# guptakhil/show-tell

Measured on AMD Instinct MI355X. Metric: training images/sec (ResNet101+GRU, emb=512, bs=128) at 1/2/4/8 MI355X, higher is better.
Workload: dtype bf16; 1 GPU; BASELINE configs[1]: ResNet-101 (train-mode BN, frozen) + 5-layer GRU decoder, E=H=512, V=10000, fwd+bwd+SGD step, synthetic COCO-shaped batch; batch_per_gpu=128, global_batch=128, image=3x224x224, parallelism=dp1

## Files before the change

### include/showtell_hip.h

```cpp
#ifndef SHOWTELL_HIP_H
#define SHOWTELL_HIP_H

#include <stddef.h>
#include <stdint.h>

#ifdef __cplusplus
extern "C" {
#endif

#define ST_F32 0
#define ST_BF16 1

#define ST_CELL_GRU 0
#define ST_CELL_LSTM 1

const char* st_last_error(void);
int st_version(void);

typedef struct {
  const void* x;
  const void* w;
  void* y;
  const float* bias;
  const float* scale;
// ... 110 lines not shown
  const void* x_s2d; const void* w_frag; void* y;
  float* stats; int stats_replicas;
  const float* gamma;
  const float* scale; const float* shift;
  int B, H, W;
} st_stem_conv_pool_desc;
int st_stem_conv_pool(const st_stem_conv_pool_desc* d, void* stream);
int st_stem_weight_frag(const void* w_s2d, void* out, void* stream);
int st_stem_weight_frag_packed(const void* w_packed, int Cpad, void* out, void* stream);
int st_global_avgpool(const void* x, void* y, int dtype, int out_dtype, int B, int HW, int C, void* stream);

typedef struct st_image_batch_desc {
  const uint8_t* src;
  int64_t src_bytes;
  const int64_t* offset;
  const int32_t* height;
  const int32_t* width;
  const int32_t* flip;
  int batch;
  int max_height, max_width;
  int out_h, out_w;
  const float* lut;
  uint8_t* tmp;
  float* out;
  uint8_t* out_u8;
} st_image_batch_desc;
int st_image_transform(const st_image_batch_desc* d, void* stream);

int st_cast(const void* x, void* y, int from_dtype, int to_dtype, long n, void* stream);
int st_transpose(const void* x, void* y, int dtype, int rows, int cols, int ldx, int ldy, void* stream);
int st_transpose_colsum(const void* x, void* y, float* colsum, int dtype, int rows, int cols, int ldx, int ldy, void* stream);
int st_transpose_batch(const void* const* x, void* const* y, float* const* colsum, int n, int dtype, int rows, int cols,
                       int ldx, int ldy, const int* rows_t, const int* prev_row, void* stream);
int st_pack_conv_weight(const float* w, void* out, int dtype, int Cout, int Cin, int KH, int KW, int Cpad, int k_order, void* stream);

typedef struct st_resnet st_resnet;
int st_resnet_create(int version, int dtype, st_resnet** out);
void st_resnet_destroy(st_resnet* r);
int st_resnet_num_convs(const st_resnet* r);
int st_resnet_feat_dim(const st_resnet* r);
size_t st_resnet_weight_elems(const st_resnet* r);
size_t st_resnet_bn_channels(const st_resnet* r);
int st_resnet_conv_info(const st_resnet* r, int i, int* cin, int* cout, int* k, int* stride, int* pad,
                        int* cin_padded, size_t* weight_offset, size_t* bn_offset, int* k_order,
                        size_t* frag_weight_offset, int* frag_ntw);
size_t st_resnet_workspace_bytes(const st_resnet* r, int B, int H, int W);
int st_resnet_set_taps(st_resnet* r, void* buf, size_t bytes);
int st_resnet_forward(const st_resnet* r, const float* images_nchw, int B, int H, int W,
                      const void* weights, const float* bn_gamma, const float* bn_beta,
                      float* bn_running_mean, float* bn_running_var,
                      int train, float momentum, float eps,
                      void* workspace, size_t workspace_bytes,
                      void* feat_nhwc_out, void* pooled_out, int pooled_dtype, float* ncp_out,
                      void* stream);

int st_resnet_update_running(const st_resnet* r, const void* workspace, float* bn_running_mean, float* bn_running_var,
                             float momentum, void* stream);
int st_resnet_plan(const st_resnet* r, int B, int H, int W, int train, char* buf, size_t bytes);

int st_cast2d(const void* x, void* y, int from_dtype, int to_dtype, int rows, int cols, int ldx, int ldy, void* stream);

#define ST_MAX_LAYERS 8
typedef struct {
  int cell, dtype, L, in0, H, V, E;
  const void* emb;
  const void* w_ih[ST_MAX_LAYERS]; const void* w_hh[ST_MAX_LAYERS];
// ... 115 lines not shown
```

### show-tell_amd/_lib.py

```python
import ctypes as C
import os

_HERE = os.path.dirname(os.path.abspath(__file__))
LIB_PATH = os.path.join(_HERE, "lib", "libshowtell_hip.so")

ST_F32, ST_BF16 = 0, 1
ST_CELL_GRU, ST_CELL_LSTM = 0, 1

c_p, c_i, c_f, c_l = C.c_void_p, C.c_int, C.c_float, C.c_long


class ConvDesc(C.Structure):
    _fields_ = [("x", c_p), ("w", c_p), ("y", c_p), ("bias", c_p), ("scale", c_p), ("shift", c_p),
                ("residual", c_p), ("stats", c_p), ("dtype", c_i), ("out_dtype", c_i),
                ("B", c_i), ("Hin", c_i), ("Win", c_i), ("Cin", c_i), ("Ho", c_i), ("Wo", c_i), ("N", c_i),
                ("KH", c_i), ("KW", c_i), ("stride", c_i), ("pad", c_i),
                ("ldx", c_i), ("ldw", c_i), ("ldy", c_i), ("relu", c_i), ("accumulate", c_i), ("Cin_logical", c_i), ("k_order", c_i), ("stats_replicas", c_i),
                ("in_stats", c_p), ("in_gamma", c_p), ("in_beta", c_p), ("in_count", c_f), ("in_eps", c_f), ("split_k", c_i)]


class Conv3x3ImgDesc(C.Structure):
    _fields_ = [("x", c_p), ("w_frag", c_p), ("y", c_p), ("stats", c_p), ("stats_replicas", c_i), ("scale", c_p), ("shift", c_p),
                ("relu", c_i), ("in_stats", c_p), ("in_gamma", c_p), ("in_beta", c_p), ("in_count", c_f), ("in_eps", c_f),
                ("B", c_i), ("H", c_i), ("W", c_i), ("C", c_i), ("N", c_i), ("in_stats_replicas", c_i)]
# ... 43 lines not shown
                ("res_beta", c_p), ("res_running_mean", c_p), ("res_running_var", c_p), ("res_bn", c_i),
                ("dtype", c_i), ("rows", c_l), ("C", c_i), ("count", c_f), ("eps", c_f), ("relu", c_i),
                ("stats_replicas", c_i), ("res_stats_replicas", c_i)]


ST_MAX_LAYERS = 8


class RnnParams(C.Structure):
    _fields_ = [("cell", c_i), ("dtype", c_i), ("L", c_i), ("in0", c_i), ("H", c_i), ("V", c_i), ("E", c_i),
                ("emb", c_p), ("w_ih", c_p * ST_MAX_LAYERS), ("w_hh", c_p * ST_MAX_LAYERS),
                ("b_ih", c_p * ST_MAX_LAYERS), ("b_hh", c_p * ST_MAX_LAYERS), ("w_lin", c_p), ("b_lin", c_p)]


class RnnGrads(C.Structure):
    _fields_ = [("emb", c_p), ("w_ih", c_p * ST_MAX_LAYERS), ("w_hh", c_p * ST_MAX_LAYERS),
                ("b_ih", c_p * ST_MAX_LAYERS), ("b_hh", c_p * ST_MAX_LAYERS), ("w_lin", c_p), ("b_lin", c_p)]


class AttnParams(C.Structure):
    _fields_ = [("rnn", RnnParams), ("F", c_i), ("A", c_i), ("P", c_i),
                ("w_enc", c_p), ("b_enc", c_p), ("w_dec", c_p), ("b_dec", c_p), ("w_full", c_p), ("b_full", c_p),
                ("w_init_h", c_p), ("b_init_h", c_p), ("w_init_c", c_p), ("b_init_c", c_p), ("w_embed", c_p), ("b_embed", c_p)]


class AttnGrads(C.Structure):
    _fields_ = [("rnn", RnnGrads)] + [(n, c_p) for n in ("w_enc", "b_enc", "w_dec", "b_dec", "w_full", "b_full", "w_init_h", "b_init_h",
                                                        "w_init_c", "b_init_c", "w_embed", "b_embed")]


class PackedSeq(C.Structure):
    _fields_ = [("B", c_i), ("T", c_i), ("ntok", c_i), ("Tcap", c_i), ("batch_sizes_host", C.POINTER(c_i)),
                ("rows_b", c_p), ("rows_t", c_p), ("prev_row", c_p), ("caption", c_p)]


class ImageBatchDesc(C.Structure):
    _fields_ = [("src", c_p), ("src_bytes", C.c_int64), ("offset", c_p), ("height", c_p), ("width", c_p), ("flip", c_p), ("batch", c_i),
                ("max_height", c_i), ("max_width", c_i), ("out_h", c_i), ("out_w", c_i), ("lut", c_p), ("tmp", c_p),
                ("out", c_p), ("out_u8", c_p)]


_SIGS = {
    "st_version": ([], c_i),
    "st_image_transform": ([C.POINTER(ImageBatchDesc), c_p], c_i),
    "st_conv": ([C.POINTER(ConvDesc), c_p], c_i),
    "st_conv_batch": ([C.POINTER(ConvDesc), c_i, c_p], c_i),
    "st_conv3x3_img_supported": ([c_i, c_i, c_i, c_i], c_i),
    "st_conv3x3_img": ([C.POINTER(Conv3x3ImgDesc), c_p], c_i),
    "st_conv3x3_s2_supported": ([c_i, c_i], c_i),
    "st_conv3x3_s2": ([C.POINTER(Conv3x3ImgDesc), c_p], c_i),
    "st_conv1x1_wreg_supported": ([c_i, c_i], c_i),
    "st_conv1x1_wreg": ([C.POINTER(Conv1x1WregDesc), c_p], c_i),
    "st_conv1x1_kfuse": ([C.POINTER(Conv1x1KfuseDesc), c_p], c_i),
    "st_conv1x1_kfuse_supported": ([c_i, c_i], c_i),
    "st_conv1x1_kfuse8": ([C.POINTER(Conv1x1KfuseDesc), c_p], c_i),
    "st_conv_b2b": ([C.POINTER(ConvB2bDesc), c_p], c_i),
    "st_conv_b2b_supported": ([c_i, c_i, c_i], c_i),
    "st_conv1x1_astat_supported": ([c_i, c_i], c_i),
    "st_conv1x1_astat": ([C.POINTER(Conv1x1WregDesc), c_p], c_i),
    "st_conv1x1_kstream_supported": ([c_i, c_i], c_i),
    "st_conv1x1_kstream": ([C.POINTER(Conv1x1WregDesc), c_p], c_i),
    "st_pack_conv_weight_frag": ([c_p, c_p, c_i, c_i, c_i, c_i, c_i, c_p], c_i),
    "st_tune": ([c_i, c_i, c_i], c_i),
    "st_prof_enable": ([c_i], c_i),
    "st_debug_stamps": ([c_p], c_i),
    "st_prof_collect": ([C.POINTER(C.c_double), C.POINTER(C.c_double), C.POINTER(c_l)], c_i),
    "st_bn_act": ([C.POINTER(BnActDesc), c_p], c_i),
    "st_bn_update_running": ([c_p, c_p, c_p, c_i, c_f, c_f, c_p], c_i),
    "st_nchw_to_nhwc": ([c_p, c_p, c_i, c_i, c_i, c_i, c_i, c_i, c_p], c_i),
    "st_nchw_to_s2d16": ([c_p, c_p, c_i, c_i, c_i, c_i, c_p], c_i),
    "st_stem_weight_s2d": ([c_p, c_p, c_i, c_i, c_p], c_i),
    "st_stem_weight_frag": ([c_p, c_p, c_p], c_i),
    "st_stem_weight_frag_packed": ([c_p, c_i, c_p, c_p], c_i),
    "st_stem_conv_pool": ([C.POINTER(StemConvPoolDesc), c_p], c_i),
    "st_nhwc_to_ncp_f32": ([c_p, c_p, c_i, c_i, c_i, c_i, c_p], c_i),
    "st_maxpool3x3s2": ([c_p, c_p, c_i, c_i, c_i, c_i, c_i, c_p], c_i),
    "st_maxpool3x3s2_bn": ([c_p, c_p, c_i, c_i, c_i, c_i, c_i, c_p, c_p, c_p, c_p, c_p, c_f, c_f, c_p], c_i),
    "st_global_avgpool": ([c_p, c_p, c_i, c_i, c_i, c_i, c_i, c_p], c_i),
    "st_cast": ([c_p, c_p, c_i, c_i, c_l, c_p], c_i),
    "st_transpose": ([c_p, c_p, c_i, c_i, c_i, c_i, c_i, c_p], c_i),
    "st_transpose_colsum": ([c_p, c_p, c_p, c_i, c_i, c_i, c_i, c_i, c_p], c_i),
    "st_transpose_batch": ([c_p, c_p, c_p, c_i, c_i, c_i, c_i, c_i, c_i, c_p, c_p, c_p], c_i),
    "st_pack_conv_weight": ([c_p, c_p, c_i, c_i, c_i, c_i, c_i, c_i, c_i, c_p], c_i),
    "st_cast2d": ([c_p, c_p, c_i, c_i, c_i, c_i, c_i, c_i, c_p], c_i),
    "st_rnn_vocab_ld": ([c_i], c_i),
    "st_rnn_workspace_bytes": ([C.POINTER(RnnParams), C.POINTER(PackedSeq)], C.c_size_t),
    "st_rnn_forward": ([C.POINTER(RnnParams), C.POINTER(PackedSeq), c_p, c_p, c_p, C.c_size_t, c_p, c_i, c_i, c_p, c_i, c_p], c_i),
    "st_rnn_fused_loss_supported": ([C.POINTER(RnnParams)], c_i),
    "st_rnn_fused_loss_bytes": ([C.POINTER(RnnParams), C.POINTER(PackedSeq)], C.c_size_t),
    "st_rnn_fused_loss": ([C.POINTER(RnnParams), C.POINTER(PackedSeq), c_p, C.c_size_t, c_p, c_p, C.c_size_t, c_p, c_p], c_i),
    "st_rnn_fused_dlogits": ([C.POINTER(RnnParams), C.POINTER(PackedSeq), c_p, C.c_size_t, c_p, c_p, c_p, c_p, c_i, c_p], c_i),
    "st_rnn_backward": ([C.POINTER(RnnParams), C.POINTER(RnnGrads), C.POINTER(PackedSeq), c_p, c_p, c_i, c_p, c_p, C.c_size_t,
                         c_p, c_p, c_p], c_i),
    "st_rnn_greedy_workspace_bytes": ([C.POINTER(RnnParams), c_i], C.c_size_t),
    "st_rnn_greedy": ([C.POINTER(RnnParams), c_p, c_i, c_i, c_p, C.c_size_t, c_p, c_p, c_p], c_i),
    "st_rnn_greedy_last_route": ([], c_i),
    "st_rnn_step": ([C.POINTER(RnnParams), c_p, c_i, c_p, c_p, c_p, c_p, c_p, c_i, c_p], c_i),
    "st_embedding_rows": ([c_p, c_p, c_p, c_i, c_i, c_i, c_i, c_i, c_p], c_i),
    "st_gather_state": ([c_p, c_p, c_p, c_i, c_i, c_i, c_i, c_i, c_p], c_i),
    "st_softmax_topk": ([c_p, c_i, c_i, c_i, c_i, c_p, c_p, c_i, c_p], c_i),
    "st_beam_select": ([c_p, c_p, c_p, c_p, c_p, c_i, c_i, c_i, c_l, c_p, c_p, c_p, c_p, c_p, c_p], c_i),
    "st_sample_rows": ([c_p, c_i, c_i, c_i, c_p, c_i, c_f, c_i, c_l, c_p, c_p, c_p, c_i, c_i, c_p, c_p], c_i),
    "st_rnn_sample_workspace_bytes": ([C.POINTER(RnnParams), c_i], C.c_size_t),
    "st_rnn_sample": ([C.POINTER(RnnParams), c_p, c_i, c_i, c_p, c_f, c_i, c_l, c_p, C.c_size_t, c_p, c_p, c_p], c_i),
    "st_attn_workspace_bytes": ([c_p, c_p], C.c_size_t),
    "st_attn_forward": ([c_p, c_p, c_p, c_p, c_p, C.c_size_t, c_p, c_i, c_i, c_p, c_i, c_p], c_i),
    "st_attn_backward": ([c_p, c_p, c_p, c_p, c_p, c_i, c_p, c_p, c_f, c_p, c_p, C.c_size_t, c_p], c_i),
    "st_attn_reg_loss": ([c_p, c_i, c_i, c_i, c_f, c_p, c_p], c_i),
    "st_attn_greedy_workspace_bytes": ([c_p, c_i], C.c_size_t),
    "st_attn_greedy": ([c_p, c_p, c_i, c_i, c_l, c_p, C.c_size_t, c_p, c_p], c_i),
    "st_attn_greedy_alphas": ([c_p, c_p, c_i, c_i, c_l, c_p, C.c_size_t, c_p, c_p, c_p], c_i),
    "st_attn_sample_workspace_bytes": ([c_p, c_i], C.c_size_t),
    "st_attn_sample": ([c_p, c_p, c_i, c_i, c_l, c_p, c_f, c_i, c_l, c_p, C.c_size_t, c_p, c_p, c_p, c_p], c_i),
    "st_attn_beam_workspace_bytes": ([c_p, c_i, c_i], C.c_size_t),
    "st_attn_beam_search": ([c_p, c_p, c_i, c_i, c_i, c_l, c_l, c_p, C.c_size_t, c_p, c_p, c_p, c_p, c_p, c_p], c_i),
# ... 63 lines not shown
```

### show-tell_amd/csrc/rnn.cpp

```cpp
#include "decoder_host.h"
#include <stdlib.h>

namespace {

struct Plan {
  int G, GH, Np, Vp, maxw;
  size_t es;
  size_t x0, y, gates, cst, dyl, dx0, dgx, dgh, dhc, dcc, tA, tB, wT, wThh, wTih, gA, gB, total;
};

Plan make_plan(const st_rnn_params* p, const st_packed_seq* s) {
  Plan q;
  q.G = p->cell == ST_CELL_GRU ? 3 : 4;
  q.GH = q.G * p->H;
  q.Np = st_up8(s->ntok);
  q.Vp = st_rnn_vocab_ld(p->V);
  q.es = st_dtype_size(p->dtype);
  q.maxw = p->in0 > p->H ? p->in0 : p->H;
  const size_t n = s->ntok, L = p->L, H = p->H;
  Arena ar;
  q.x0 = ar.take(n * p->in0 * q.es);
  q.y = ar.take(L * n * H * q.es);
  q.gates = ar.take(L * n * 4 * H * q.es);
  q.cst = ar.take(p->cell == ST_CELL_LSTM ? L * n * H * q.es : 0);
  q.dyl = ar.take(L * n * H * sizeof(float));
  q.dx0 = ar.take(n * p->in0 * sizeof(float));
  q.dgx = ar.take(L * n * q.GH * q.es);
  q.dgh = ar.take(p->cell == ST_CELL_GRU ? L * n * q.GH * q.es : 0);
  q.dhc = ar.take(L * (size_t)s->B * H * sizeof(float));
  q.dcc = ar.take(L * (size_t)s->B * H * sizeof(float));
  const size_t ra = (size_t)(p->V > q.GH ? p->V : q.GH);
  q.tA = ar.take(ra * q.Np * q.es);
  q.tB = ar.take((size_t)q.maxw * q.Np * q.es);
  const size_t w1 = (size_t)H * q.Vp, w2 = (size_t)q.maxw * q.GH;
  q.wT = ar.take((w1 > w2 ? w1 : w2) * q.es);
  q.wThh = ar.take(L * H * q.GH * q.es);
  q.wTih = ar.take(L * (size_t)q.maxw * q.GH * q.es);
  q.gA = ar.take(2 * L * (size_t)q.GH * q.Np * q.es);
  q.gB = ar.take(2 * L * (size_t)q.maxw * q.Np * q.es);
  q.total = ar.o;
  return q;
}

int check_common(const st_rnn_params* p, const st_packed_seq* s, const char* who) {
  ST_CHECK(p && s, "%s: null descriptor", who);
  ST_CHECK(p->cell == ST_CELL_GRU || p->cell == ST_CELL_LSTM, "%s: bad cell %d", who, p->cell);
  ST_CHECK(p->dtype == ST_F32 || p->dtype == ST_BF16, "%s: bad dtype %d", who, p->dtype);
  ST_CHECK(p->L >= 1 && p->L <= ST_MAX_LAYERS, "%s: num_layers=%d out of range [1,%d]", who, p->L, ST_MAX_LAYERS);
  ST_CHECK(p->H % 8 == 0 && p->in0 % 8 == 0 && p->E % 8 == 0, "%s: E=%d, in0=%d and H=%d must be multiples of 8", who, p->E, p->in0, p->H);
  ST_CHECK(p->V > 0, "%s: bad vocabulary size", who);
  if (st_check_packed_seq(s, who, true)) return 1;
  for (int l = 0; l < p->L; ++l)
    ST_CHECK(p->w_ih[l] && p->w_hh[l] && p->b_ih[l] && p->b_hh[l], "%s: null weights for layer %d", who, l);
  return 0;
}

}

extern "C" int st_rnn_vocab_ld(int V) { return V < 2048 ? st_up8(V) : (V + 511) / 512 * 512; }

extern "C" size_t st_rnn_workspace_bytes(const st_rnn_params* p, const st_packed_seq* s) {
  if (!p || !s) return 0;
  return make_plan(p, s).total;
}

extern "C" int st_rnn_forward(const st_rnn_params* p, const st_packed_seq* s, const void* x0_override, const void* feat,
                              void* workspace, size_t workspace_bytes, void* logits, int logits_dtype, int ldl,
                              long* targets, int save_for_backward, void* stream) {
  if (check_common(p, s, "st_rnn_forward")) return 1;
  ST_CHECK(workspace && (x0_override || (feat && p->emb)), "st_rnn_forward: null pointer");
  const Plan q = make_plan(p, s);
  ST_CHECK(workspace_bytes >= q.total, "st_rnn_forward: workspace too small (%zu < %zu)", workspace_bytes, q.total);
  hipStream_t st = reinterpret_cast<hipStream_t>(stream);
  char* ws = reinterpret_cast<char*>(workspace);
  const int dt = p->dtype, H = p->H, n = s->ntok;
  const size_t es = q.es;
// ... 50 lines not shown
  const int n = s->ntok;
  return vocab_ce_forward(ytop, p->w_lin, p->b_lin, targets, n, p->V, scratch + 2 * (size_t)n, scratch + n, scratch, loss_accum,
                          reinterpret_cast<hipStream_t>(stream));
}
extern "C" int st_rnn_fused_dlogits(const st_rnn_params* p, const st_packed_seq* s, const void* workspace, size_t workspace_bytes,
                                    const long* targets, const float* scratch, const float* grad_scale_dev, void* dlogits, int ldd, void* stream) {
  if (check_common(p, s, "st_rnn_fused_dlogits")) return 1;
  ST_CHECK(workspace && targets && scratch && dlogits, "st_rnn_fused_dlogits: null pointer");
  ST_CHECK(st_rnn_fused_loss_supported(p), "st_rnn_fused_dlogits: unsupported configuration");
  const Plan q = make_plan(p, s);
  ST_CHECK(workspace_bytes >= q.total, "st_rnn_fused_dlogits: workspace too small");
  const char* ytop = reinterpret_cast<const char*>(workspace) + q.y + (size_t)(p->L - 1) * s->ntok * p->H * q.es;
  return vocab_ce_dlogits(ytop, p->w_lin, p->b_lin, targets, scratch, s->ntok, p->V, dlogits, ldd, 1.0f, grad_scale_dev,
                          reinterpret_cast<hipStream_t>(stream));
}

extern "C" int st_rnn_backward(const st_rnn_params* p, const st_rnn_grads* g, const st_packed_seq* s,
                               const void* x0_override, const void* dlogits, int ldd, const float* dy_top_extra,
                               void* workspace, size_t workspace_bytes, float* dfeat, float* dx0_out, void* stream) {
  if (check_common(p, s, "st_rnn_backward")) return 1;
  ST_CHECK(g && workspace, "st_rnn_backward: null pointer");
  const Plan q = make_plan(p, s);
  ST_CHECK(workspace_bytes >= q.total, "st_rnn_backward: workspace too small (%zu < %zu)", workspace_bytes, q.total);
  hipStream_t st = reinterpret_cast<hipStream_t>(stream);
  char* ws = reinterpret_cast<char*>(workspace);
  const int dt = p->dtype, H = p->H, n = s->ntok, Np = q.Np, GH = q.GH;
  const size_t es = q.es;
  const std::vector<int> off = st_packed_offsets(s);
  const int L = p->L, T = s->T;
  auto dyl = [&](int l) { return reinterpret_cast<float*>(ws + q.dyl) + (size_t)l * n * H; };
  float* dy = dyl(L - 1);
  const char* ytop = ws + q.y + (size_t)(p->L - 1) * n * H * es;

  if (dlogits) {
    ST_CHECK(p->w_lin && g->w_lin && g->b_lin, "st_rnn_backward: vocabulary projection gradients requested without buffers");
    ST_CHECK(ldd >= st_up8(p->V) && ldd % 8 == 0 && ldd <= q.Vp, "st_rnn_backward: dlogits leading dimension %d must be a multiple of 8 in [%d, %d]",
             ldd, st_up8(p->V), q.Vp);
    if (st_transpose_colsum(dlogits, ws + q.tA, g->b_lin, dt, n, p->V, ldd, Np, stream)) return 1;
    if (st_transpose(ytop, ws + q.tB, dt, n, H, H, Np, stream)) return 1;
    if (st_gemm_nt(ws + q.tA, Np, ws + q.tB, Np, g->w_lin, H, p->V, H, Np, dt, ST_F32, nullptr, stream, 1)) return 1;
    if (st_transpose(p->w_lin, ws + q.wT, dt, p->V, H, H, ldd, stream)) return 1;
    const int bk = dt == ST_BF16 ? 64 : 32;
    const int split = (ldd % (8 * bk) == 0 && ldd >= 16 * bk) ? 8 : 0;
    if (st_gemm_nt(dlogits, ldd, ws + q.wT, ldd, dy, H, n, H, ldd, dt, ST_F32, nullptr, stream, 0, split)) return 1;
    if (dy_top_extra) { st_set_error("st_rnn_backward: dlogits and dy_top_extra are exclusive"); return 1; }
  } else {
    ST_CHECK(dy_top_extra, "st_rnn_backward: need dlogits or dy_top");
    if (hipMemcpyAsync(dy, dy_top_extra, (size_t)n * H * sizeof(float), hipMemcpyDeviceToDevice, st) != hipSuccess) {
      st_set_error("st_rnn_backward: copy failed"); return 1;
    }
  }

  const void* x0 = x0_override ? x0_override : ws + q.x0;
  const bool need_dx0 = dfeat || dx0_out || g->emb;
  float* dx0 = dx0_out ? dx0_out : reinterpret_cast<float*>(ws + q.dx0);
  const bool gru = p->cell == ST_CELL_GRU;
  auto dgxl = [&](int l) { return ws + q.dgx + (size_t)l * n * GH * es; };
  auto dghl = [&](int l) { return gru ? ws + q.dgh + (size_t)l * n * GH * es : dgxl(l); };
  auto dhcl = [&](int l) { return reinterpret_cast<float*>(ws + q.dhc) + (size_t)l * s->B * H; };
  auto dccl = [&](int l) { return reinterpret_cast<float*>(ws + q.dcc) + (size_t)l * s->B * H; };
  auto wThh = [&](int l) { return ws + q.wThh + (size_t)l * H * GH * es; };
  auto wTih = [&](int l) { return ws + q.wTih + (size_t)l * q.maxw * GH * es; };
  if (hipMemsetAsync(ws + q.dhc, 0, (size_t)L * s->B * H * sizeof(float), st) != hipSuccess ||
      hipMemsetAsync(ws + q.dcc, 0, (size_t)L * s->B * H * sizeof(float), st) != hipSuccess) { st_set_error("memset failed"); return 1; }
  {
    const void* wx[2][ST_MAX_LAYERS]; void* wy[2][ST_MAX_LAYERS];
    int ni = 0;
    for (int l = 0; l < L; ++l) {
      const int in = l == 0 ? p->in0 : H;
      wx[0][l] = p->w_hh[l]; wy[0][l] = wThh(l);
      if (!(l > 0 || need_dx0)) continue;
      if (in == H) { wx[1][ni] = p->w_ih[l]; wy[1][ni] = wTih(l); ++ni; }
      else if (st_transpose(p->w_ih[l], wTih(l), dt, GH, in, in, GH, stream)) return 1;
    }
    if (st_transpose_batch(wx[0], wy[0], nullptr, L, dt, GH, H, H, GH, nullptr, nullptr, stream)) return 1;
    if (ni && st_transpose_batch(wx[1], wy[1], nullptr, ni, dt, GH, H, H, GH, nullptr, nullptr, stream)) return 1;
  }
  auto bwd_cell = [&](int l, int t, const float* dyrows) {
    const char* yl = ws + q.y + (size_t)l * n * H * es;
    const char* gl = ws + q.gates + (size_t)l * n * 4 * H * es;
    const char* cl = ws + q.cst + (size_t)l * n * H * es;
    RnnBwdCell c;
    memset(&c, 0, sizeof(c));
    c.dy = dyrows ? dyrows + (size_t)off[t] * H : nullptr; c.dhc = dhcl(l); c.dcc = dccl(l);
    c.cache = gl + (size_t)off[t] * 4 * H * es;
    c.hprev = t > 0 ? yl + (size_t)off[t - 1] * H * es : nullptr;
    c.cnew = cl + (size_t)off[t] * H * es;
    c.cprev = t > 0 ? cl + (size_t)off[t - 1] * H * es : nullptr;
    c.dgx = dgxl(l) + (size_t)off[t] * GH * es; c.dgh = dghl(l) + (size_t)off[t] * GH * es; c.Bt = s->batch_sizes_host[t];
    return c;
  };
  const char* env = getenv("ST_BPTT_FUSED");
  const bool fused = !(env && env[0] == '0');
  for (int d = T + L - 2; fused && d >= 0; --d) {
    RnnBwdFused fc[ST_MAX_LAYERS];
    int nf = 0;
    for (int l = d < T ? 0 : d - (T - 1); l <= d && l < L; ++l) {
      const int t = d - l;
      RnnBwdFused& f = fc[nf++];
      memset(&f, 0, sizeof(f));
      f.e = bwd_cell(l, t, l == L - 1 ? dy : nullptr);
      RnnGemmArgs& a = f.g;
      a.M = f.e.Bt; a.N = H;
      if (t + 1 < T) {
        a.A = dghl(l) + (size_t)off[t + 1] * GH * es; a.W = wThh(l); a.M2 = s->batch_sizes_host[t + 1]; a.K = GH; a.lda = GH; a.ldw = GH;
      }
      if (l + 1 < L) {
        a.A2 = dgxl(l + 1) + (size_t)off[t] * GH * es; a.W2 = wTih(l + 1); a.K2 = GH; a.lda2 = GH; a.ldw2 = GH;
      }
    }
    if (rnn_bwd_fused_launch_batch(fc, nf, p->cell, dt, st)) return 1;
  }
  if (fused && need_dx0 && st_gemm_nt(dgxl(0), GH, wTih(0), GH, dx0, p->in0, n, p->in0, GH, dt, ST_F32, nullptr, stream)) return 1;
  for (int d = T + L - 2; !fused && d >= 0; --d) {
    RnnBwdCell gc[ST_MAX_LAYERS];
    RnnGemmArgs mc[2 * ST_MAX_LAYERS];
    int ng = 0, nm = 0;
    for (int l = d < T ? 0 : d - (T - 1); l <= d && l < L; ++l) {
      const int t = d - l;
      const int bt = s->batch_sizes_host[t];
      const int in = l == 0 ? p->in0 : H;
      gc[ng++] = bwd_cell(l, t, dyl(l));
      if (t > 0) {
        RnnGemmArgs& a = mc[nm++];
        memset(&a, 0, sizeof(a));
        a.A = dghl(l) + (size_t)off[t] * GH * es; a.W = wThh(l); a.M = bt; a.N = H; a.K = GH; a.lda = GH; a.ldw = GH;
        a.out_f32 = dhcl(l); a.ldo = H; a.accumulate = 1;
      }
      if (l > 0 || need_dx0) {
        RnnGemmArgs& a = mc[nm++];
        memset(&a, 0, sizeof(a));
        a.A = dgxl(l) + (size_t)off[t] * GH * es; a.W = wTih(l); a.M = bt; a.N = in; a.K = GH; a.lda = GH; a.ldw = GH;
        a.out_f32 = (l > 0 ? dyl(l - 1) + (size_t)off[t] * H : dx0 + (size_t)off[t] * in); a.ldo = in;
      }
    }
    if (rnn_bwd_gates_launch_batch(gc, ng, H, p->cell, dt, st)) return 1;
    if (rnn_gemm_launch_batch(mc, nm, dt, 0, 0, st)) return 1;
  }
  st_conv_desc gd[2 * ST_MAX_LAYERS];
  int ng = 0;
  auto wgrad = [&](const void* aT, const void* bT, float* dw, int rows, int cols) {
    gd[ng++] = st_gemm_nt_desc(aT, Np, bT, Np, dw, cols, rows, cols, Np, dt, ST_F32, nullptr, 1);
  };
  const void* tx[4][ST_MAX_LAYERS]; void* ty[4][ST_MAX_LAYERS]; float* tc[4][ST_MAX_LAYERS];
  int nx = 0;
  for (int l = 0; l < L; ++l) {
    const int in = l == 0 ? p->in0 : H;
    const char* xl = l == 0 ? reinterpret_cast<const char*>(x0) : ws + q.y + (size_t)(l - 1) * n * H * es;
    char* aIh = ws + q.gA + (size_t)(2 * l) * GH * Np * es;
    char* aHh = ws + q.gA + (size_t)(2 * l + 1) * GH * Np * es;
    char* bIh = ws + q.gB + (size_t)(2 * l) * q.maxw * Np * es;
    char* bHh = ws + q.gB + (size_t)(2 * l + 1) * q.maxw * Np * es;
    tx[0][l] = dgxl(l); ty[0][l] = aIh; tc[0][l] = g->b_ih[l];
    tx[2][l] = dghl(l); ty[2][l] = aHh; tc[2][l] = g->b_hh[l];
    tx[3][l] = ws + q.y + (size_t)l * n * H * es; ty[3][l] = bHh; tc[3][l] = nullptr;
    if (in == H) {
      tx[1][nx] = xl; ty[1][nx] = bIh; tc[1][nx] = nullptr; ++nx;
      wgrad(aIh, bIh, g->w_ih[l], GH, in);
    } else {
      if (st_transpose(xl, bIh, dt, n, in, in, Np, stream)) return 1;
    }
    wgrad(gru ? aHh : aIh, bHh, g->w_hh[l], GH, H);
    if (!gru && colsum_launch(dghl(l), g->b_hh[l], n, GH, GH, dt, st)) return 1;
  }
  if (st_transpose_batch(tx[0], ty[0], tc[0], L, dt, n, GH, GH, Np, nullptr, nullptr, stream)) return 1;
  if (nx && st_transpose_batch(tx[1], ty[1], nullptr, nx, dt, n, H, H, Np, nullptr, nullptr, stream)) return 1;
  if (gru && st_transpose_batch(tx[2], ty[2], tc[2], L, dt, n, GH, GH, Np, nullptr, nullptr, stream)) return 1;
  if (st_transpose_batch(tx[3], ty[3], nullptr, L, dt, n, H, H, Np, s->rows_t, s->prev_row, stream)) return 1;
  for (int l = 0; l < L; ++l) {
    const int in = l == 0 ? p->in0 : H;
// ... 13 lines not shown
```

Before: 32030 images/sec.

## Add row-major bf16 GEMM kernel to skip transposes in decoder backward

Adds a batched bf16 MFMA GEMM that reads row-major operands directly, using LDS transpose reads for the TN form, fused column-sum for bias gradients, gather via prev_row for the hidden-state weight gradient, and optional split-K with atomics. The decoder backward uses it by default for the vocabulary projection gradients, the dx0 product and the per-layer weight gradients. This removes the explicit transpose kernels and their scratch traffic, and also skips transposing the layer-0 input weights. The cost is a new hand-written kernel whose tile choice and atomic split-K may be less tuned than the existing GEMM path. The decoder backward is a small share of a ResNet-101 training step.

```diff
diff --git a/include/showtell_hip.h b/include/showtell_hip.h
--- a/include/showtell_hip.h
+++ b/include/showtell_hip.h
@@ -166,6 +166,21 @@
 int st_transpose_colsum(const void* x, void* y, float* colsum, int dtype, int rows, int cols, int ldx, int ldy, void* stream);
 int st_transpose_batch(const void* const* x, void* const* y, float* const* colsum, int n, int dtype, int rows, int cols,
                        int ldx, int ldy, const int* rows_t, const int* prev_row, void* stream);
+typedef struct {
+  const void* a;
+  const void* b;
+  float* c;
+  float* colsum;
+  const int* rows_t;
+  const int* prev_row;
+  int M, N, K, lda, ldb, ldc;
+  int trans_a;
+  int accumulate;
+  int split_k;
+  int tile;
+} st_gemm_rm_desc;
+int st_gemm_rm(const st_gemm_rm_desc* d, int n, void* stream);
+
 int st_pack_conv_weight(const float* w, void* out, int dtype, int Cout, int Cin, int KH, int KW, int Cpad, int k_order, void* stream);
 
 typedef struct st_resnet st_resnet;
diff --git a/show-tell_amd/_lib.py b/show-tell_amd/_lib.py
--- a/show-tell_amd/_lib.py
+++ b/show-tell_amd/_lib.py
@@ -99,6 +99,12 @@
 class PackedSeq(C.Structure):
     _fields_ = [("B", c_i), ("T", c_i), ("ntok", c_i), ("Tcap", c_i), ("batch_sizes_host", C.POINTER(c_i)),
                 ("rows_b", c_p), ("rows_t", c_p), ("prev_row", c_p), ("caption", c_p)]
+
+
+class GemmRmDesc(C.Structure):
+    _fields_ = [("a", c_p), ("b", c_p), ("c", c_p), ("colsum", c_p), ("rows_t", c_p), ("prev_row", c_p),
+                ("M", c_i), ("N", c_i), ("K", c_i), ("lda", c_i), ("ldb", c_i), ("ldc", c_i),
+                ("trans_a", c_i), ("accumulate", c_i), ("split_k", c_i), ("tile", c_i)]
 
 
 class ImageBatchDesc(C.Structure):
@@ -148,6 +154,7 @@
     "st_transpose": ([c_p, c_p, c_i, c_i, c_i, c_i, c_i, c_p], c_i),
     "st_transpose_colsum": ([c_p, c_p, c_p, c_i, c_i, c_i, c_i, c_i, c_p], c_i),
     "st_transpose_batch": ([c_p, c_p, c_p, c_i, c_i, c_i, c_i, c_i, c_i, c_p, c_p, c_p], c_i),
+    "st_gemm_rm": ([C.POINTER(GemmRmDesc), c_i, c_p], c_i),
     "st_pack_conv_weight": ([c_p, c_p, c_i, c_i, c_i, c_i, c_i, c_i, c_i, c_p], c_i),
     "st_cast2d": ([c_p, c_p, c_i, c_i, c_i, c_i, c_i, c_i, c_p], c_i),
     "st_rnn_vocab_ld": ([c_i], c_i),
diff --git a/show-tell_amd/csrc/gemm_rm.hip b/show-tell_amd/csrc/gemm_rm.hip
--- /dev/null
+++ b/show-tell_amd/csrc/gemm_rm.hip
@@ -0,0 +1,294 @@
+#include "common.h"
+#include <stdlib.h>
+#include <string.h>
+
+namespace {
+
+constexpr int kBK = 32;
+constexpr int kMaxBatch = 12;
+constexpr int kDepth = 4;
+
+struct GemmRmBatch {
+  const bf16_t* a[kMaxBatch]; const bf16_t* b[kMaxBatch]; float* c[kMaxBatch]; float* colsum[kMaxBatch];
+  const int* rows_t[kMaxBatch]; const int* prev_row[kMaxBatch];
+};
+
+typedef __attribute__((ext_vector_type(4))) short s16x4;
+typedef __attribute__((address_space(3))) s16x4 lds_s16x4;
+
+__device__ __forceinline__ s16x4 lds_read_tr(const bf16_t* p) {
+  return __builtin_amdgcn_ds_read_tr16_b64_v4i16((lds_s16x4*)(p));
+}
+__device__ __forceinline__ bf16x8 frag_of(s16x4 lo, s16x4 hi) {
+  typedef __attribute__((ext_vector_type(8))) short s16x8;
+  const s16x8 v = __builtin_shufflevector(lo, hi, 0, 1, 2, 3, 4, 5, 6, 7);
+  return __builtin_bit_cast(bf16x8, v);
+}
+
+template <int BM, int BN, bool TA, bool GATHER>
+__global__ __launch_bounds__(256, 2) void gemm_rm_kernel(GemmRmBatch gb, int M, int N, int K, int lda, int ldb, int ldc,
+                                                         int accumulate, int slices, int steps_per_slice) {
+  constexpr int PA = TA ? BM + 16 : kBK + 8;
+  constexpr int PB = BN + 16;
+  constexpr int SZA = TA ? kBK * PA : BM * PA, SZB = kBK * PB;
+  constexpr int CPA = TA ? BM / 8 : kBK / 8;
+  constexpr int CPB = BN / 8;
+  constexpr int NLA = (TA ? kBK : BM) * CPA / 256, NLB = kBK * CPB / 256;
+  constexpr int RSA = 256 / CPA, RSB = 256 / CPB;
+  constexpr int MT = BM / 32, NT = BN / 32;
+  static_assert(NLA >= 1 && NLB >= 1, "tile too small for 256 threads");
+  __shared__ __attribute__((aligned(16))) bf16_t lds[2 * (SZA + SZB)];
+  static_assert(2 * (SZA + SZB) * 2 >= (256 / (BM / 8)) * BM * 4 || !TA, "column-sum scratch does not fit");
+
+  const int nbx = (N + BN - 1) / BN, nby = (M + BM - 1) / BM;
+  const int total = gridDim.x, lin = blockIdx.x;
+  const int xcd = lin & 7, q8 = total >> 3, r8 = total & 7;
+  int id = xcd * q8 + (xcd < r8 ? xcd : r8) + (lin >> 3);
+  const int bx = id % nbx; id /= nbx;
+  const int by = id % nby, bz = id / nby;
+  const int prob = bz / slices, slice = bz - prob * slices;
+  const bf16_t* __restrict__ A = gb.a[prob];
+  const bf16_t* __restrict__ B = gb.b[prob];
+  float* __restrict__ C = gb.c[prob];
+  float* __restrict__ colsum = gb.colsum[prob];
+  const bool has_tab = GATHER && gb.rows_t[prob] != nullptr;
+  const int* __restrict__ tab_t = has_tab ? gb.rows_t[prob] : reinterpret_cast<const int*>(B);
+  const int* __restrict__ tab_p = has_tab ? gb.prev_row[prob] : reinterpret_cast<const int*>(B);
+  const int m0 = by * BM, n0 = bx * BN;
+  const int tid = threadIdx.x, lane = tid & 63, wid = tid >> 6;
+  const int wm = (wid >> 1) * (BM / 2), wn = (wid & 1) * (BN / 2);
+  const int g = lane >> 4, i16 = lane & 15;
+
+  const int nsteps = (K + kBK - 1) / kBK;
+  const int s0 = slice * steps_per_slice;
+  const int s1 = s0 + steps_per_slice < nsteps ? s0 + steps_per_slice : nsteps;
+
+  const bool do_colsum = TA && colsum != nullptr && bx == 0;
+  float cs[8];
+#pragma unroll
+  for (int e = 0; e < 8; ++e) cs[e] = 0.f;
+
+  const int arow = tid / CPA, acol = (tid % CPA) * 8;
+  const int brow = tid / CPB, bcol = (tid % CPB) * 8;
+  const bool a_in = !TA || m0 + acol < M, b_in = n0 + bcol < N;
+
+  constexpr int D = kDepth;
+  u32x4 rra[D][NLA], rrb[D][NLB];
+  unsigned okm[D];
+  int gt[D][NLB], gp[D][NLB];
+  auto fetch_tab = [&](int (&t)[NLB], int (&p)[NLB], int step) {
+#pragma unroll
+    for (int i = 0; i < NLB; ++i) {
+      int k = step * kBK + brow + i * RSB;
+      k = k < K ? k : K - 1;
+      t[i] = tab_t[k]; p[i] = tab_p[k];
+    }
+  };
+  auto fetch = [&](u32x4 (&ra)[NLA], u32x4 (&rb)[NLB], unsigned& ok, const int (&t)[NLB], const int (&p)[NLB], int step) {
+    const int k0 = step * kBK;
+    ok = 0u;
+#pragma unroll
+    for (int i = 0; i < NLA; ++i) {
+      const int r = arow + i * RSA;
+      const bool in = TA ? (k0 + r < K && a_in) : (m0 + r < M && k0 + acol < K);
+      const long o = TA ? (long)(k0 + r) * lda + m0 + acol : (long)(m0 + r) * lda + k0 + acol;
+      ra[i] = *reinterpret_cast<const u32x4*>(A + (in ? o : 0));
+      ok |= (unsigned)in << i;
+    }
+#pragma unroll
+    for (int i = 0; i < NLB; ++i) {
+      const int k = k0 + brow + i * RSB;
+      bool in = k < K && b_in;
+      long sr = k;
+      if (GATHER) { in = in && (!has_tab || t[i] > 0); sr = has_tab ? p[i] : k; }
+      rb[i] = *reinterpret_cast<const u32x4*>(B + (in ? sr * ldb + n0 + bcol : 0));
+      ok |= (unsigned)in << (8 + i);
+    }
+  };
+  auto stash = [&](const u32x4 (&ra)[NLA], const u32x4 (&rb)[NLB], unsigned ok, int buf, int step) {
+    bf16_t* la = lds + buf * (SZA + SZB);
+    bf16_t* lb = la + SZA;
+    const u32x4 zero = {0u, 0u, 0u, 0u};
+#pragma unroll
+    for (int i = 0; i < NLA; ++i) {
+      u32x4 v = (ok >> i) & 1u ? ra[i] : zero;
+      if (!TA) {
+        const int left = K - (step * kBK + acol);
+#pragma unroll
+        for (int e = 0; e < 4; ++e) v[e] &= left >= 2 * e + 2 ? 0xffffffffu : (left == 2 * e + 1 ? 0xffffu : 0u);
+      }
+      *reinterpret_cast<u32x4*>(la + (arow + i * RSA) * PA + acol) = v;
+      if (do_colsum) {
+#pragma unroll
+        for (int e = 0; e < 4; ++e) {
+          cs[2 * e] += __uint_as_float(v[e] << 16);
+          cs[2 * e + 1] += __uint_as_float(v[e] & 0xffff0000u);
+        }
+      }
+    }
+#pragma unroll
+    for (int i = 0; i < NLB; ++i)
+      *reinterpret_cast<u32x4*>(lb + (brow + i * RSB) * PB + bcol) = (ok >> (8 + i)) & 1u ? rb[i] : zero;
+  };
+
+  f32x4 acc[MT][NT];
+#pragma unroll
+  for (int t = 0; t < MT; ++t)
+#pragma unroll
+    for (int u = 0; u < NT; ++u) acc[t][u] = f32x4{0.f, 0.f, 0.f, 0.f};
+
+  const int tr_row = 4 * g + (i16 >> 2), tr_col = 4 * (i16 & 3);
+  const int offA = TA ? tr_row * PA + wm + tr_col : (wm + i16) * PA + 4 * g;
+  const int offB = tr_row * PB + wn + tr_col;
+
+#pragma unroll
+  for (int j = 0; j < D; ++j) {
+    if (GATHER) fetch_tab(gt[j], gp[j], s0 + j);
+    else { for (int i = 0; i < NLB; ++i) gt[j][i] = gp[j][i] = 0; }
+  }
+#pragma unroll
+  for (int j = 0; j < D; ++j) fetch(rra[j], rrb[j], okm[j], gt[j], gp[j], s0 + j);
+  if (GATHER) {
+#pragma unroll
+    for (int j = 0; j < D; ++j) fetch_tab(gt[j], gp[j], s0 + D + j);
+  }
+  stash(rra[0], rrb[0], okm[0], 0, s0);
+  __syncthreads();
+  for (int base = s0; base < s1; base += D) {
+#pragma unroll
+    for (int j = 0; j < D; ++j) {
+      const int step = base + j;
+      if (step >= s1) break;
+      fetch(rra[j], rrb[j], okm[j], gt[j], gp[j], step + D);
+      if (GATHER) fetch_tab(gt[j], gp[j], step + 2 * D);
+      const bf16_t* la = lds + (j & 1) * (SZA + SZB);
+      const bf16_t* lb = la + SZA;
+      bf16x8 fa[MT], fb[NT];
+#pragma unroll
+      for (int t = 0; t < MT; ++t) {
+        if (TA) {
+          fa[t] = frag_of(lds_read_tr(la + offA + t * 16), lds_read_tr(la + offA + t * 16 + 16 * PA));
+        } else {
+          const bf16_t* p = la + offA + t * 16 * PA;
+          fa[t] = frag_of(*reinterpret_cast<const s16x4*>(p), *reinterpret_cast<const s16x4*>(p + 16));
+        }
+      }
+#pragma unroll
+      for (int u = 0; u < NT; ++u) fb[u] = frag_of(lds_read_tr(lb + offB + u * 16), lds_read_tr(lb + offB + u * 16 + 16 * PB));
+#pragma unroll
+      for (int t = 0; t < MT; ++t)
+#pragma unroll
+        for (int u = 0; u < NT; ++u) acc[t][u] = __builtin_amdgcn_mfma_f32_16x16x32_bf16(fa[t], fb[u], acc[t][u], 0, 0, 0);
+      stash(rra[(j + 1) % D], rrb[(j + 1) % D], okm[(j + 1) % D], (j + 1) & 1, step + 1);
+      __syncthreads();
+    }
+  }
+
+  float cold[MT][4][NT];
+#pragma unroll
+  for (int t = 0; t < MT; ++t)
+#pragma unroll
+    for (int r = 0; r < 4; ++r)
+#pragma unroll
+      for (int u = 0; u < NT; ++u) {
+        const int m = m0 + wm + t * 16 + 4 * g + r, n = n0 + wn + u * 16 + i16;
+        const bool in = m < M && n < N && accumulate && slices == 1;
+        cold[t][r][u] = C[in ? (long)m * ldc + n : 0];
+      }
+#pragma unroll
+  for (int t = 0; t < MT; ++t)
+#pragma unroll
+    for (int r = 0; r < 4; ++r) {
+      const int m = m0 + wm + t * 16 + 4 * g + r;
+#pragma unroll
+      for (int u = 0; u < NT; ++u) {
+        const int n = n0 + wn + u * 16 + i16;
+        if (m >= M || n >= N) continue;
+        float* p = C + (long)m * ldc + n;
+        if (slices > 1) atomicAdd(p, acc[t][u][r]);
+        else *p = accumulate ? cold[t][r][u] + acc[t][u][r] : acc[t][u][r];
+      }
+    }
+
+  if (TA && do_colsum) {
+    constexpr int RG = 256 / (BM / 8);
+    float* red = reinterpret_cast<float*>(lds);
+#pragma unroll
+    for (int e = 0; e < 8; ++e) red[(tid / CPA) * BM + (tid % CPA) * 8 + e] = cs[e];
+    __syncthreads();
+    if (tid < BM && m0 + tid < M) {
+      float s = 0.f;
+#pragma unroll 8
+      for (int r = 0; r < RG; ++r) s += red[r * BM + tid];
+      atomicAdd(colsum + m0 + tid, s);
+    }
+  }
+}
+
+template <int BM, int BN, bool TA, bool GATHER>
+void launch_rm(const GemmRmBatch& gb, const st_gemm_rm_desc& d, int n, int slices, int sps, hipStream_t st) {
+  const dim3 grid(((d.N + BN - 1) / BN) * ((d.M + BM - 1) / BM) * n * slices);
+  hipLaunchKernelGGL((gemm_rm_kernel<BM, BN, TA, GATHER>), grid, dim3(256), 0, st, gb, d.M, d.N, d.K, d.lda, d.ldb, d.ldc, d.accumulate, slices, sps);
+}
+template <int BM, int BN>
+void launch_rm(const GemmRmBatch& gb, const st_gemm_rm_desc& d, int n, bool gather, int slices, int sps, hipStream_t st) {
+  if (d.trans_a) {
+    if (gather) launch_rm<BM, BN, true, true>(gb, d, n, slices, sps, st);
+    else launch_rm<BM, BN, true, false>(gb, d, n, slices, sps, st);
+  } else {
+    if (gather) launch_rm<BM, BN, false, true>(gb, d, n, slices, sps, st);
+    else launch_rm<BM, BN, false, false>(gb, d, n, slices, sps, st);
+  }
+}
+
+}
+
+extern "C" int st_gemm_rm(const st_gemm_rm_desc* d, int n, void* stream) {
+  ST_CHECK(d && n >= 1 && n <= kMaxBatch, "st_gemm_rm: 1..12 problems per launch");
+  const st_gemm_rm_desc& f = d[0];
+  ST_CHECK(f.M >= 1 && f.N >= 1 && f.K >= 1, "st_gemm_rm: empty product (M=%d N=%d K=%d)", f.M, f.N, f.K);
+  ST_CHECK(f.lda % 8 == 0 && f.ldb % 8 == 0, "st_gemm_rm: lda=%d and ldb=%d must be multiples of 8", f.lda, f.ldb);
+  ST_CHECK(f.lda >= (f.trans_a ? f.M : f.K) && f.ldb >= f.N && f.ldc >= f.N, "st_gemm_rm: leading dimension too small (lda=%d ldb=%d ldc=%d)",
+           f.lda, f.ldb, f.ldc);
+  ST_CHECK(f.tile == 0 || f.tile == 64 || f.tile == 128, "st_gemm_rm: tile must be 0 (chosen here), 64 or 128");
+  ST_CHECK(f.split_k <= 1 || !f.trans_a, "st_gemm_rm: split_k is for the NN form only (weight gradients stay free of atomics)");
+  GemmRmBatch gb;
+  memset(&gb, 0, sizeof(gb));
+  bool gather = false;
+  for (int i = 0; i < n; ++i) {
+    const st_gemm_rm_desc& e = d[i];
+    ST_CHECK(e.a && e.b && e.c, "st_gemm_rm: null pointer (problem %d)", i);
+    ST_CHECK(((reinterpret_cast<uintptr_t>(e.a) | reinterpret_cast<uintptr_t>(e.b)) & 15) == 0, "st_gemm_rm: a and b must be 16-byte aligned (problem %d)", i);
+    ST_CHECK((e.rows_t == nullptr) == (e.prev_row == nullptr), "st_gemm_rm: rows_t and prev_row go together");
+    ST_CHECK(!e.colsum || e.trans_a, "st_gemm_rm: colsum needs the TN form");
+    ST_CHECK(e.M == f.M && e.N == f.N && e.K == f.K && e.lda == f.lda && e.ldb == f.ldb && e.ldc == f.ldc && e.trans_a == f.trans_a &&
+             e.accumulate == f.accumulate && e.split_k == f.split_k && e.tile == f.tile, "st_gemm_rm: the problems of one launch must have one shape and one set of options");
+    gb.a[i] = reinterpret_cast<const bf16_t*>(e.a); gb.b[i] = reinterpret_cast<const bf16_t*>(e.b); gb.c[i] = e.c; gb.colsum[i] = e.colsum;
+    gb.rows_t[i] = e.rows_t; gb.prev_row[i] = e.prev_row;
+    gather = gather || e.rows_t;
+  }
+  hipStream_t st = reinterpret_cast<hipStream_t>(stream);
+  const int nsteps = (f.K + kBK - 1) / kBK;
+  int slices = 1, sps = nsteps;
+  if (f.split_k > 1 && nsteps >= f.split_k) {
+    sps = (nsteps + f.split_k - 1) / f.split_k;
+    slices = (nsteps + sps - 1) / sps;
+  }
+  if (slices > 1 && !f.accumulate) {
+    for (int i = 0; i < n; ++i) {
+      if (hipMemset2DAsync(d[i].c, (size_t)f.ldc * sizeof(float), 0, (size_t)f.N * sizeof(float), f.M, st) != hipSuccess) {
+        st_set_error("st_gemm_rm: memset failed"); return 1;
+      }
+    }
+  }
+  int tile = f.tile;
+  if (!tile) {
+    const long big = (long)((f.M + 127) / 128) * ((f.N + 127) / 128) * n * slices;
+    const long slots = (big + 255) / 256 * 256;
+    tile = big >= 256 && 4 * big >= 3 * slots ? 128 : 64;
+  }
+  if (tile == 128) launch_rm<128, 128>(gb, f, n, gather, slices, sps, st);
+  else launch_rm<64, 64>(gb, f, n, gather, slices, sps, st);
+  ST_LAUNCH_CHECK();
+  return 0;
+}
diff --git a/show-tell_amd/csrc/rnn.cpp b/show-tell_amd/csrc/rnn.cpp
--- a/show-tell_amd/csrc/rnn.cpp
+++ b/show-tell_amd/csrc/rnn.cpp
@@ -42,6 +42,15 @@
   return q;
 }
 
+st_gemm_rm_desc rm_desc(const void* a, int lda, int trans_a, const void* b, int ldb, float* c, int ldc, int M, int N, int K,
+                        int accumulate, float* colsum = nullptr, int split_k = 0) {
+  st_gemm_rm_desc d;
+  memset(&d, 0, sizeof(d));
+  d.a = a; d.b = b; d.c = c; d.colsum = colsum; d.M = M; d.N = N; d.K = K; d.lda = lda; d.ldb = ldb; d.ldc = ldc;
+  d.trans_a = trans_a; d.accumulate = accumulate; d.split_k = split_k;
+  return d;
+}
+
 int check_common(const st_rnn_params* p, const st_packed_seq* s, const char* who) {
   ST_CHECK(p && s, "%s: null descriptor", who);
   ST_CHECK(p->cell == ST_CELL_GRU || p->cell == ST_CELL_LSTM, "%s: bad cell %d", who, p->cell);
@@ -158,18 +167,27 @@
   float* dy = dyl(L - 1);
   const char* ytop = ws + q.y + (size_t)(p->L - 1) * n * H * es;
 
+  const char* env_rm = getenv("ST_DEC_GEMM_RM");
+  const bool rm = dt == ST_BF16 && !(env_rm && env_rm[0] == '0');
   if (dlogits) {
     ST_CHECK(p->w_lin && g->w_lin && g->b_lin, "st_rnn_backward: vocabulary projection gradients requested without buffers");
     ST_CHECK(ldd >= st_up8(p->V) && ldd % 8 == 0 && ldd <= q.Vp, "st_rnn_backward: dlogits leading dimension %d must be a multiple of 8 in [%d, %d]",
              ldd, st_up8(p->V), q.Vp);
-    if (st_transpose_colsum(dlogits, ws + q.tA, g->b_lin, dt, n, p->V, ldd, Np, stream)) return 1;
-    if (st_transpose(ytop, ws + q.tB, dt, n, H, H, Np, stream)) return 1;
-    if (st_gemm_nt(ws + q.tA, Np, ws + q.tB, Np, g->w_lin, H, p->V, H, Np, dt, ST_F32, nullptr, stream, 1)) return 1;
-    if (st_transpose(p->w_lin, ws + q.wT, dt, p->V, H, H, ldd, stream)) return 1;
     const int bk = dt == ST_BF16 ? 64 : 32;
     const int split = (ldd % (8 * bk) == 0 && ldd >= 16 * bk) ? 8 : 0;
-    if (st_gemm_nt(dlogits, ldd, ws + q.wT, ldd, dy, H, n, H, ldd, dt, ST_F32, nullptr, stream, 0, split)) return 1;
     if (dy_top_extra) { st_set_error("st_rnn_backward: dlogits and dy_top_extra are exclusive"); return 1; }
+    if (rm) {
+      const st_gemm_rm_desc dw = rm_desc(dlogits, ldd, 1, ytop, H, g->w_lin, H, p->V, H, n, 1, g->b_lin);
+      if (st_gemm_rm(&dw, 1, stream)) return 1;
+      const st_gemm_rm_desc dyt = rm_desc(dlogits, ldd, 0, p->w_lin, H, dy, H, n, H, p->V, 0, nullptr, split);
+      if (st_gemm_rm(&dyt, 1, stream)) return 1;
+    } else {
+      if (st_transpose_colsum(dlogits, ws + q.tA, g->b_lin, dt, n, p->V, ldd, Np, stream)) return 1;
+      if (st_transpose(ytop, ws + q.tB, dt, n, H, H, Np, stream)) return 1;
+      if (st_gemm_nt(ws + q.tA, Np, ws + q.tB, Np, g->w_lin, H, p->V, H, Np, dt, ST_F32, nullptr, stream, 1)) return 1;
+      if (st_transpose(p->w_lin, ws + q.wT, dt, p->V, H, H, ldd, stream)) return 1;
+      if (st_gemm_nt(dlogits, ldd, ws + q.wT, ldd, dy, H, n, H, ldd, dt, ST_F32, nullptr, stream, 0, split)) return 1;
+    }
   } else {
     ST_CHECK(dy_top_extra, "st_rnn_backward: need dlogits or dy_top");
     if (hipMemcpyAsync(dy, dy_top_extra, (size_t)n * H * sizeof(float), hipMemcpyDeviceToDevice, st) != hipSuccess) {
@@ -181,21 +199,23 @@
   const bool need_dx0 = dfeat || dx0_out || g->emb;
   float* dx0 = dx0_out ? dx0_out : reinterpret_cast<float*>(ws + q.dx0);
   const bool gru = p->cell == ST_CELL_GRU;
+  const char* env = getenv("ST_BPTT_FUSED");
+  const bool fused = !(env && env[0] == '0');
   auto dgxl = [&](int l) { return ws + q.dgx + (size_t)l * n * GH * es; };
   auto dghl = [&](int l) { return gru ? ws + q.dgh + (size_t)l * n * GH * es : dgxl(l); };
   auto dhcl = [&](int l) { return reinterpret_cast<float*>(ws + q.dhc) + (size_t)l * s->B * H; };
   auto dccl = [&](int l) { return reinterpret_cast<float*>(ws + q.dcc) + (size_t)l * s->B * H; };
   auto wThh = [&](int l) { return ws + q.wThh + (size_t)l * H * GH * es; };
   auto wTih = [&](int l) { return ws + q.wTih + (size_t)l * q.maxw * GH * es; };
-  if (hipMemsetAsync(ws + q.dhc, 0, (size_t)L * s->B * H * sizeof(float), st) != hipSuccess ||
-      hipMemsetAsync(ws + q.dcc, 0, (size_t)L * s->B * H * sizeof(float), st) != hipSuccess) { st_set_error("memset failed"); return 1; }
+  const size_t carry = (size_t)L * s->B * H * sizeof(float);
+  if (hipMemsetAsync(ws + q.dhc, 0, gru ? carry : q.dcc - q.dhc + carry, st) != hipSuccess) { st_set_error("memset failed"); return 1; }
   {
     const void* wx[2][ST_MAX_LAYERS]; void* wy[2][ST_MAX_LAYERS];
     int ni = 0;
     for (int l = 0; l < L; ++l) {
       const int in = l == 0 ? p->in0 : H;
       wx[0][l] = p->w_hh[l]; wy[0][l] = wThh(l);
-      if (!(l > 0 || need_dx0)) continue;
+      if (!(l > 0 || need_dx0) || (l == 0 && fused && rm)) continue;
       if (in == H) { wx[1][ni] = p->w_ih[l]; wy[1][ni] = wTih(l); ++ni; }
       else if (st_transpose(p->w_ih[l], wTih(l), dt, GH, in, in, GH, stream)) return 1;
     }
@@ -216,8 +236,6 @@
     c.dgx = dgxl(l) + (size_t)off[t] * GH * es; c.dgh = dghl(l) + (size_t)off[t] * GH * es; c.Bt = s->batch_sizes_host[t];
     return c;
   };
-  const char* env = getenv("ST_BPTT_FUSED");
-  const bool fused = !(env && env[0] == '0');
   for (int d = T + L - 2; fused && d >= 0; --d) {
     RnnBwdFused fc[ST_MAX_LAYERS];
     int nf = 0;
@@ -237,7 +255,10 @@
     }
     if (rnn_bwd_fused_launch_batch(fc, nf, p->cell, dt, st)) return 1;
   }
-  if (fused && need_dx0 && st_gemm_nt(dgxl(0), GH, wTih(0), GH, dx0, p->in0, n, p->in0, GH, dt, ST_F32, nullptr, stream)) return 1;
+  if (fused && need_dx0 && rm) {
+    const st_gemm_rm_desc d0 = rm_desc(dgxl(0), GH, 0, p->w_ih[0], p->in0, dx0, p->in0, n, p->in0, GH, 0);
+    if (st_gemm_rm(&d0, 1, stream)) return 1;
+  } else if (fused && need_dx0 && st_gemm_nt(dgxl(0), GH, wTih(0), GH, dx0, p->in0, n, p->in0, GH, dt, ST_F32, nullptr, stream)) return 1;
   for (int d = T + L - 2; !fused && d >= 0; --d) {
     RnnBwdCell gc[ST_MAX_LAYERS];
     RnnGemmArgs mc[2 * ST_MAX_LAYERS];
@@ -262,6 +283,28 @@
     }
     if (rnn_bwd_gates_launch_batch(gc, ng, H, p->cell, dt, st)) return 1;
     if (rnn_gemm_launch_batch(mc, nm, dt, 0, 0, st)) return 1;
+  }
+  if (rm) {
+    st_gemm_rm_desc rd[2 * ST_MAX_LAYERS];
+    int nr = 0;
+    for (int l = 0; l < L; ++l) {
+      const int in = l == 0 ? p->in0 : H;
+      const char* xl = l == 0 ? reinterpret_cast<const char*>(x0) : ws + q.y + (size_t)(l - 1) * n * H * es;
+      const st_gemm_rm_desc ih = rm_desc(dgxl(l), GH, 1, xl, in, g->w_ih[l], in, GH, in, n, 1, g->b_ih[l]);
+      if (in == H) rd[nr++] = ih;
+      else if (st_gemm_rm(&ih, 1, stream)) return 1;
+      st_gemm_rm_desc hh = rm_desc(dghl(l), GH, 1, ws + q.y + (size_t)l * n * H * es, H, g->w_hh[l], H, GH, H, n, 1, g->b_hh[l]);
+      hh.rows_t = s->rows_t; hh.prev_row = s->prev_row;
+      rd[nr++] = hh;
+    }
+    for (int i = 0; i < nr; i += 12) {
+      if (st_gemm_rm(rd + i, nr - i < 12 ? nr - i : 12, stream)) return 1;
+    }
+    if (need_dx0 && !x0_override) {
+      ST_CHECK(g->emb, "st_rnn_backward: embedding gradient buffer missing");
+      if (embedding_bwd_launch(dx0, s->caption, s->Tcap, s->rows_b, s->rows_t, dfeat, g->emb, n, p->E, p->V, 0, st)) return 1;
+    }
+    return 0;
   }
   st_conv_desc gd[2 * ST_MAX_LAYERS];
   int ng = 0;
```

Result: no change. 32350 images/sec, median of 6 (+1.0%).
